# qiaozhijian/VCR-Net

Hardware: AMD Instinct MI355X
Metric: point-cloud pairs/sec (N=1024, batch 16 per GPU) (higher is better)
Workload: dtype f32; 1 GPU; BASELINE configs[1]: ModelNet40-like whole-to-whole registration, N=1024, batch=16 pairs per GPU, LPDNet(k=20)+Transformer+VcpTopK+SVD, iter=1, fp32; synthetic object clouds with the reference's transform recipe; LPD-pretrained emb_nn + seeded Transformer weights; num_points=1024, batch_per_gpu=16, global_batch=16, k=20, iters=1, parallelism=dp1 (pairs sharded per rank), entry_point=vcrnet_amd.module.vcrnetIter(net, src, tgt, iter) -> vcr_vcrnet_iter_f32

## Files before the change

### include/vcr_hip.h

```cpp
#ifndef VCR_HIP_H
#define VCR_HIP_H

#include <stddef.h>
#include <stdint.h>

#ifdef __cplusplus
extern "C" {
#endif

#define VCR_OK 0
#define VCR_EINVAL (-1)
#define VCR_EWORKSPACE (-2)
#define VCR_EUNSUPPORTED (-3)

typedef void* vcr_stream_t;

const char* vcr_strerror(int code);
#define VCR_ABI_VERSION 27
int vcr_abi_version(void);

typedef struct {
  const float* x_cf; int B, N;
  const float* w1; const float* b1;
  const float* w2; const float* b2;
  float* xyz4; float* feat64; float* sq64;
  const float* x_cf2; int B2;
  const float* pq_w; const float* pq_b; float* pq; int ldpq;
  float* feat64t;
} vcr_pointwise_args;
int vcr_pointwise_f32(const vcr_pointwise_args*, vcr_stream_t);

int vcr_rows4_f32(const float* x_cf, float* xyz4, int B, int N, vcr_stream_t);
int vcr_rows4_pq_f32(const float* x_cf, float* xyz4, int B, int N, const float* wpq, int ldw, const float* bpq, int C,
                     float* pq, int ldpq, vcr_stream_t);

typedef struct {
  uint32_t struct_bytes;
  const float* x; int ldx;
  const float* sq;
  int B, N, C, k;
  int32_t* idx;
  int32_t* tie_scratch; int tie_cap;
  int waves;
  int tie_zeroed;
  int tie_defer;
  void* tie_work; size_t tie_work_bytes;
  int tie_inline;
  const float* xt;
  const int32_t* perm; const float* xp; const float* sqp;
  const float* cen; const float* cen_sq; const float* cen_rad; const float* cen_sqmax;
  const int32_t* ord_ok;
} vcr_knn_args;

typedef struct {
  const float* xyz4;
  const float* feat_t; int ldf; const float* sq;
  int B, N;
  int32_t* perm; float* xyz4_p; float* cen4; float* cen4_rad; float* cen4_sqmax;
  float* feat_p; float* sq_p; float* cen64; float* cen64_sq; float* cen64_rad; float* cen64_sqmax;
  int32_t* ord_ok; float* ord_stat; float guard_ratio;
} vcr_knn_order_args;
int vcr_knn_order_f32(const vcr_knn_order_args*, vcr_stream_t);
int vcr_knn_f32(const vcr_knn_args*, vcr_stream_t);
size_t vcr_knn_tie_work_bytes(int N);
size_t vcr_knn_tie_slot_bytes(int B, int N);
int vcr_knn_ties_inline(const vcr_knn_args*);
int vcr_knn_ties_f32(const vcr_knn_args* a, const vcr_knn_args* b, vcr_stream_t);
int vcr_knn_pair_f32(const vcr_knn_args* a64, const vcr_knn_args* a3, vcr_stream_t);

typedef struct {
  const float* x; int ldx;
  const float* w;
  const float* bias;
  const float* residual; int ldr;
  float* y; int ldy;
  int M, N, K;
  int relu;
  const float* ln_stats_in; int ln_nseg; const float* ln_colsum; float ln_eps;
  float* stats_out;
  float* segmax_out; int ld_segmax; int seg_k;
  int variant;
} vcr_linear_args;
enum {
  VCR_LINEAR_REGSTAGE = 4, VCR_LINEAR_BK32 = 8, VCR_LINEAR_MFMA16 = 16, VCR_LINEAR_BK16 = 64, VCR_LINEAR_MFMA32 = 1024,
  VCR_LINEAR_ROWS96 = 2048, VCR_LINEAR_ROWS128 = 4096, VCR_LINEAR_ROWS64 = 8192, VCR_LINEAR_ROWS32 = 16384
};
int vcr_linear_f32(const vcr_linear_args*, vcr_stream_t);
int vcr_linear_config(const vcr_linear_args*);
int vcr_linear_pair_f32(const vcr_linear_args* a, const vcr_linear_args* b, vcr_stream_t);

int vcr_fold_layernorm_f32(const float* w, const float* bias, const float* ln_a, const float* ln_b, int N, int K,
                           float* w_out, float* colsum, float* bias_out, vcr_stream_t);

int vcr_split_bf16x3_f32(const float* x, void* planes, size_t n, vcr_stream_t);
int vcr_linear_bf16x3_f32(const vcr_linear_args*, const void* w_planes, vcr_stream_t);

typedef struct {
  const float* x; int ldx; const float* a; const float* b; float eps;
  const float* residual; int ldr;
  float* y; int ldy; int M, C;
  const float* xyz4; float* side4;
} vcr_layernorm_args;
int vcr_layernorm_f32(const vcr_layernorm_args*, vcr_stream_t);

typedef struct {
  const float* x; int ldx; int M, C; float scale; float* y; int ldy;
  const float* xyz4; float* side4;
} vcr_rowside_args;
int vcr_rowside_f32(const vcr_rowside_args*, vcr_stream_t);

typedef struct {
  const float* pq; int ldpq; const int32_t* idx; int k; int M; int n_per_cloud;
  const float* w2; const float* b2;
  float* x1; int ldx1; float* x2; int ldx2;
} vcr_edgeconv_args;
int vcr_edgeconv_f32(const vcr_edgeconv_args*, vcr_stream_t);
int vcr_edgeconv_bf16x3_f32(const vcr_edgeconv_args*, vcr_stream_t);

typedef struct {
  const float* pq; int ldpq; int C; const int32_t* idx; int k; int M; int n_per_cloud;
  float* y; int ldy;
  int variant;
  const int32_t* order;
} vcr_gathermax_args;
int vcr_gathermax_f32(const vcr_gathermax_args*, vcr_stream_t);

typedef struct {
  const float* pq; int ldpq; int C; const int32_t* idx; int k; int M; int n_per_cloud; float* h; int ldh;
  float* ymax; int ldymax; int zero_to;
} vcr_edgerows_args;
int vcr_edgerows_f32(const vcr_edgerows_args*, vcr_stream_t);
typedef struct {
  const float* pq; int ldpq; const int32_t* idx; int k; int M; int n_per_cloud;
  const float *w2, *b2, *w3, *b3, *w4, *b4;
  float* out; int ldo;
} vcr_edgechain_args;
int vcr_edgechain_f32(const vcr_edgechain_args*, vcr_stream_t);
typedef struct {
  const float* x; int ldx; int M, k, C; float* y; int ldy;
} vcr_segmax_args;
int vcr_segmax_f32(const vcr_segmax_args*, vcr_stream_t);

typedef struct {
  const float* q; int ldq; const float* k; int ldk; const float* v; int ldv;
  float* out; int ldo;
  int nbatch, heads, nq, nk; float scale; int kv_batch_shift;
  const uint8_t* key_keep; float* rowstat;
  float* score_out; int ld_score;
  int ngroups; long q_group_stride, k_group_stride, v_group_stride, out_group_stride;
  const int32_t* key_index; int nk_src;
  float* split_work; long split_work_floats;
  int variant;
  int plan_nbatch;
} vcr_sdpa_args;
#define VCR_SDPA_MAX_SPLIT 4
int vcr_sdpa_f32(const vcr_sdpa_args*, vcr_stream_t);
int vcr_sdpa_bf16x3_f32(const vcr_sdpa_args*, vcr_stream_t);

typedef struct {
  const float* score; int ld; int nbatch, heads, nq, nk;
  const float* rowstat; int q_batch_shift; float* mass;
} vcr_keymass_args;
int vcr_keymass_f32(const vcr_keymass_args*, vcr_stream_t);

typedef struct {
  const float* q; int ldq; const float* k; int ldk; const float* qside4; const float* kside4;
  float* corr4; int nbatch, nq, nk, E; int mode; float scale;
  float* split_work;
  long split_work_floats;
} vcr_softcorr_args;
int vcr_softcorr_f32(const vcr_softcorr_args*, vcr_stream_t);

typedef struct {
  const float* own; int ld_own; const float* str; int ld_str;
  const float* own_side4; const float* str_side4;
  int nbatch, n_own, n_str, E; int score; float scale; int str_batch_shift; int op;
  float* corr4; float* stat2; int32_t* argmax;
  const float* str_stat2; long str_stat_batch_stride; float* mass; int accumulate;
  float* score_out; int ld_score;
  int variant;
  float* split_work; long split_work_floats;
} vcr_pairscore_args;
#define VCR_PAIRSCORE_MAX_SPLIT 4
int vcr_pairscore_f32(const vcr_pairscore_args*, vcr_stream_t);

typedef struct {
  const float* score; int ld; int nbatch, n_rows, n_cols;
  const float* row_stat2; float* col_stat2; float* col_mass; float* row_mass;
} vcr_scoremass_args;
int vcr_scoremass_f32(const vcr_scoremass_args*, vcr_stream_t);

typedef struct {
  const float* values; int nbatch, n, K; int32_t* order; uint8_t* mask;
  int largest;
  int stride;
} vcr_rankselect_args;
int vcr_rankselect_f32(const vcr_rankselect_args*, vcr_stream_t);

typedef struct {
  const float* in; int ld_in; int n_in; const int32_t* idx; int nbatch, n_out, C; float* out; int ld_out;
  const int32_t* via; int n_via;
} vcr_gather_args;
int vcr_gather_rows_f32(const vcr_gather_args*, vcr_stream_t);

typedef struct {
  const float* src; int lds; const float* corr; int ldc; int B, K;
  float* R; float* t; float* R_ba; float* t_ba; float* H;
} vcr_rigid_svd_args;
int vcr_rigid_svd_f32(const vcr_rigid_svd_args*, vcr_stream_t);

typedef struct {
  const float* src4; const float* dst4; int B, N, M; int max_iterations; float tolerance;
  float* final4; float* R; float* t; float* R_ba; float* t_ba; int* iterations;
} vcr_icp_args;
size_t vcr_icp_workspace_bytes(int B, int N);
int vcr_icp_f32(const vcr_icp_args*, void* workspace, size_t workspace_bytes, vcr_stream_t);

typedef struct {
  const float* cloud; int P;
  const double* R_ab; const double* t_ab;
  const int32_t* pick; const int32_t* perm_src; const int32_t* perm_tgt;
  int B, N, keep;
  float* src_cf; float* tgt_cf;
} vcr_make_pairs_args;
int vcr_make_pairs_f32(const vcr_make_pairs_args*, vcr_stream_t);

typedef struct {
  uint32_t struct_bytes;
  const float* xyz_cf; long cloud_stride;
  int B, N, npoint;
  const int32_t* start;
  int32_t* idx;
  float* out_cf;
  int variant;
} vcr_fps_args;
int vcr_fps_f32(const vcr_fps_args*, vcr_stream_t);
int vcr_fps_form(const vcr_fps_args*, int* form, int* points_per_thread);

// ... 102 lines not shown
```

### vcr-net_amd/csrc/linear.hip

```cpp
#include "common.h"
#include "vcr_internal.h"
#include <type_traits>
#include <utility>

namespace {

constexpr int BM = 128, BN = 128;
constexpr int LINEAR_WG_PER_CU_BK32 = 2, LINEAR_WG_PER_CU_BK16 = 4;
constexpr int LINEAR_MS_DEFAULT = 0;


constexpr int LINEAR_BLOCKED_ACC = 0;

template <int BK> struct TileT { float a[BM][BK + 4]; float b[BN][BK + 4]; };

template <int BK>
__global__ __launch_bounds__(256, (BK == 32 ? 2 : 3)) void linear_kernel(vcr_linear_args p, int tiles_m, int tiles_n,
                                                                        int vec_epilogue) {
  using Tile = TileT<BK>;
  constexpr int CPR = BK / 4;
  constexpr int RPP = 256 / CPR;
  constexpr int NPASS = BM / RPP;
  extern __shared__ __attribute__((aligned(16))) unsigned char smem[];
  Tile* tile = reinterpret_cast<Tile*>(smem);
  const int t = threadIdx.x, lane = t & 63, wave = __builtin_amdgcn_readfirstlane(t >> 6);
  const int half = lane >> 5, l31 = lane & 31;
  const int wm = wave >> 1, wn = wave & 1;

  const int nblk = tiles_m * tiles_n;
  int bid = blockIdx.x;
  bid = xcd_chunk(bid, nblk);
  const int tm = bid / tiles_n, tn = bid % tiles_n;
  const int m0 = tm * BM, n0 = tn * BN;

  const int r0 = t / CPR, c4 = (t % CPR) * 4;
  const float* xa[NPASS];
  const float* wb[NPASS];
#pragma unroll
  for (int i = 0; i < NPASS; ++i) {
    xa[i] = p.x + (size_t)min(m0 + r0 + RPP * i, p.M - 1) * p.ldx + c4;
    wb[i] = p.w + (size_t)min(n0 + r0 + RPP * i, p.N - 1) * p.K + c4;
  }
  f32x4 ra[NPASS], rb[NPASS];
#pragma unroll
  for (int i = 0; i < NPASS; ++i) { ra[i] = ld4(xa[i]); rb[i] = ld4(wb[i]); }
#pragma unroll
  for (int i = 0; i < NPASS; ++i) { st4(&tile[0].a[r0 + RPP * i][c4], ra[i]); st4(&tile[0].b[r0 + RPP * i][c4], rb[i]); }
  __syncthreads();

  f32x16 acc[2][2];
#pragma unroll
  for (int i = 0; i < 2; ++i)
#pragma unroll
    for (int j = 0; j < 2; ++j) acc[i][j] = f32x16{0};

  f32x16 tot[2][2];
#pragma unroll
  for (int i = 0; i < 2; ++i)
#pragma unroll
    for (int j = 0; j < 2; ++j) tot[i][j] = f32x16{0};
  const int nk = p.K / BK;
  for (int kt = 0; kt < nk; ++kt) {
    const int cur = kt & 1;
    if (kt + 1 < nk) {
#pragma unroll
      for (int i = 0; i < NPASS; ++i) { ra[i] = ld4(xa[i] + (kt + 1) * BK); rb[i] = ld4(wb[i] + (kt + 1) * BK); }
    }
    const Tile& T = tile[cur];
#pragma unroll
    for (int g = 0; g < BK / 8; ++g) {
      f32x4 fa[2], fb[2];
#pragma unroll
      for (int i = 0; i < 2; ++i) fa[i] = ld4(&T.a[wm * 64 + i * 32 + l31][8 * g + 4 * half]);
#pragma unroll
      for (int j = 0; j < 2; ++j) fb[j] = ld4(&T.b[wn * 64 + j * 32 + l31][8 * g + 4 * half]);
#pragma unroll
      for (int s = 0; s < 4; ++s)
#pragma unroll
        for (int i = 0; i < 2; ++i)
#pragma unroll
          for (int j = 0; j < 2; ++j) acc[i][j] = mfma32(fa[i][s], fb[j][s], acc[i][j]);
    }
    if (LINEAR_BLOCKED_ACC && (((kt + 1) * BK) % 128 == 0 || kt + 1 == nk)) {
#pragma unroll
      for (int i = 0; i < 2; ++i)
#pragma unroll
        for (int j = 0; j < 2; ++j) { tot[i][j] += acc[i][j]; acc[i][j] = f32x16{0}; }
    }
    if (kt + 1 < nk) {
      Tile& Nx = tile[cur ^ 1];
#pragma unroll
      for (int i = 0; i < NPASS; ++i) { st4(&Nx.a[r0 + RPP * i][c4], ra[i]); st4(&Nx.b[r0 + RPP * i][c4], rb[i]); }
    }
    __syncthreads();
  }
  if (LINEAR_BLOCKED_ACC) {
#pragma unroll
    for (int i = 0; i < 2; ++i)
#pragma unroll
      for (int j = 0; j < 2; ++j) acc[i][j] = tot[i][j];
  }

  if (vec_epilogue) {
    constexpr int EP = 68;
    float* ot = reinterpret_cast<float*>(smem) + wave * 32 * EP;
    const int c4e = (lane & 15) * 4, col = n0 + wn * 64 + c4e;
    const f32x4 bias = (p.bias && col < p.N) ? ld4(p.bias + col) : f32x4{0.f, 0.f, 0.f, 0.f};
#pragma unroll
    for (int i = 0; i < 2; ++i) {
#pragma unroll
      for (int j = 0; j < 2; ++j)
#pragma unroll
        for (int r = 0; r < 16; ++r) ot[acc_row(r, half) * EP + j * 32 + l31] = acc[i][j][r];
      __builtin_amdgcn_s_waitcnt(0xc07f);
      __builtin_amdgcn_wave_barrier();
      if (col < p.N) {
#pragma unroll 4
        for (int ps = 0; ps < 8; ++ps) {
          const int rl = ps * 4 + (lane >> 4);
          const int row = m0 + wm * 64 + i * 32 + rl;
          if (row < p.M) {
            f32x4 v = ld4(&ot[rl * EP + c4e]) + bias;
            if (p.relu) v = f32x4{fmaxf(v[0], 0.f), fmaxf(v[1], 0.f), fmaxf(v[2], 0.f), fmaxf(v[3], 0.f)};
            if (p.residual) v = v + ld4(p.residual + (size_t)row * p.ldr + col);
            st4(p.y + (size_t)row * p.ldy + col, v);
          }
        }
      }
      __builtin_amdgcn_s_waitcnt(0xc07f);
      __builtin_amdgcn_wave_barrier();
    }
    return;
  }
#pragma unroll
  for (int j = 0; j < 2; ++j) {
    const int col = n0 + wn * 64 + j * 32 + l31;
    if (col >= p.N) continue;
    const float bias = p.bias ? p.bias[col] : 0.f;
#pragma unroll
    for (int i = 0; i < 2; ++i) {
#pragma unroll
      for (int r = 0; r < 16; ++r) {
        const int row = m0 + wm * 64 + i * 32 + acc_row(r, half);
        if (row < p.M) {
          float v = acc[i][j][r] + bias;
          if (p.relu) v = fmaxf(v, 0.f);
          if (p.residual) v += p.residual[(size_t)row * p.ldr + col];
          p.y[(size_t)row * p.ldy + col] = v;
        }
      }
    }
  }
}

template <int BK, int BMV = BM> struct TileGT { float a[BMV][BK]; float b[BN][BK]; };

__device__ __forceinline__ void glds16(const float* g, float* l) {
  __builtin_amdgcn_global_load_lds((const __attribute__((address_space(1))) void*)g,
                                   (__attribute__((address_space(3))) void*)l, 16, 0, 0);
}

template <int BK, int MS, int BMV = BM>
__device__ __forceinline__ void linear_glds_body(const vcr_linear_args& p, int tiles_m, int tiles_n, int blk) {
  const bool LN_IN = p.ln_stats_in != nullptr, STATS_OUT = p.stats_out != nullptr;
  static_assert(BMV == 128 || ((BMV == 96 || BMV == 64 || BMV == 32) && MS == 16), "the lower tiles are built from 16 x 16 MFMA tiles");
  using Tile = TileGT<BK, BMV>;
  constexpr int WR = BMV / 2;
  constexpr int EPR = BMV == 128 ? 32 : 16;
  constexpr int NPASS = WR / EPR, NPS = EPR / 4;
  constexpr int CPR = BK / 4;
  constexpr int RPK = 64 / CPR;
  constexpr int NF = 32 / RPK;
  constexpr int SWS = BK == 32 ? 1 : 2;
  constexpr int EP = 68;
  constexpr int STAGE_BYTES = 2 * sizeof(Tile) > 4 * 32 * EP * 4 ? 2 * sizeof(Tile) : 4 * 32 * EP * 4;
  extern __shared__ __attribute__((aligned(16))) unsigned char smem[];
  Tile* tile = reinterpret_cast<Tile*>(smem);
  float* rowst = reinterpret_cast<float*>(smem + STAGE_BYTES);
  const int t = threadIdx.x, lane = t & 63, wave = __builtin_amdgcn_readfirstlane(t >> 6);
  const int half = lane >> 5, l31 = lane & 31;
  const int wm = wave >> 1, wn = wave & 1;
  const int nblk = tiles_m * tiles_n;
  const int bid = xcd_chunk(blk, nblk);
  constexpr int GW = 12;
  const int grp = bid / (GW * tiles_m), wg = min(GW, tiles_n - grp * GW), loc = bid - grp * GW * tiles_m;
  const int tm = loc / wg, tn = grp * GW + loc % wg;
  const int m0 = tm * BMV, n0 = tn * BN;
  const int frow = lane / CPR, fpc = lane % CPR;
  constexpr int NFA = BMV == 128 ? NF : (BMV / RPK + 3) / 4;
  const float* xa[NFA];
  const float* wb[NF];
  int arow[NFA];
#pragma unroll
  for (int i = 0; i < NFA; ++i) {
    arow[i] = BMV == 128 ? wave * 32 + RPK * i : (wave + 4 * i) * RPK;
    const int row = min(arow[i], BMV - RPK) + frow;
    const int lc = fpc ^ ((row >> SWS) & (CPR - 1));
    xa[i] = p.x + (size_t)min(m0 + row, p.M - 1) * p.ldx + 4 * lc;
  }
#pragma unroll
  for (int i = 0; i < NF; ++i) {
    const int row = wave * 32 + RPK * i + frow;
    const int lc = fpc ^ ((row >> SWS) & (CPR - 1));
    wb[i] = p.w + (size_t)min(n0 + row, p.N - 1) * p.K + 4 * lc;
  }
  auto fill = [&](int buf, int k0) {
#pragma unroll
    for (int i = 0; i < NFA; ++i)
      if (BMV == 128 || arow[i] < BMV) glds16(xa[i] + k0, &tile[buf].a[min(arow[i], BMV - RPK)][0]);
#pragma unroll
    for (int i = 0; i < NF; ++i) glds16(wb[i] + k0, &tile[buf].b[wave * 32 + RPK * i][0]);
  };
  fill(0, 0);
  if (LN_IN && t < BMV) {
    float mean, var;
    ln_row_moments(p.ln_stats_in + (size_t)min(m0 + t, p.M - 1) * p.ln_nseg * 2, p.ln_nseg, p.K, mean, var);
    rowst[2 * t] = mean;
    rowst[2 * t + 1] = 1.f / (sqrtf(var) + p.ln_eps);
  }
  __syncthreads();

  constexpr int NT = MS == 32 ? 2 : 4;
  constexpr int NTM = WR / MS;
  const int qtr = lane >> 4, l15 = lane & 15;
  f32x16 acc[2][2];
  f32x4 acc4[MS == 16 ? NTM : 4][4];
#pragma unroll
  for (int i = 0; i < 2; ++i)
#pragma unroll
    for (int j = 0; j < 2; ++j) acc[i][j] = f32x16{0};
#pragma unroll
  for (int i = 0; i < (MS == 16 ? NTM : 4); ++i)
#pragma unroll
    for (int j = 0; j < 4; ++j) acc4[i][j] = f32x4{0.f, 0.f, 0.f, 0.f};
  int ra_[NT], rb_[NT], sa[NT], sb[NT];
#pragma unroll
  for (int i = 0; i < NT; ++i) {
    ra_[i] = wm * WR + i * MS + (MS == 32 ? l31 : l15); sa[i] = (ra_[i] >> SWS) & (CPR - 1);
    rb_[i] = wn * 64 + i * MS + (MS == 32 ? l31 : l15); sb[i] = (rb_[i] >> SWS) & (CPR - 1);
  }
  constexpr bool PREFETCH_RES = BK == 32;
  f32x4 resv[PREFETCH_RES ? NPASS : 1][PREFETCH_RES ? NPS : 1];
  if (PREFETCH_RES) {
    const int colr = n0 + wn * 64 + (lane & 15) * 4;
#pragma unroll
    for (int i = 0; i < NPASS; ++i)
#pragma unroll
      for (int ps = 0; ps < NPS; ++ps) {
        const int row = m0 + wm * WR + i * EPR + ps * 4 + (lane >> 4);
        resv[PREFETCH_RES ? i : 0][PREFETCH_RES ? ps : 0] =
            (p.residual && row < p.M && colr < p.N) ? ld4(p.residual + (size_t)row * p.ldr + colr) : f32x4{0.f, 0.f, 0.f, 0.f};
      }
  }
  constexpr bool BLOCKED = LINEAR_BLOCKED_ACC == 1 || (LINEAR_BLOCKED_ACC == 2 && BK == 32);
  f32x16 tot[BLOCKED ? 2 : 1][BLOCKED ? 2 : 1];
  f32x4 tot4[BLOCKED ? (MS == 16 ? NTM : 4) : 1][BLOCKED ? 4 : 1];
  if constexpr (BLOCKED) {
#pragma unroll
    for (int i = 0; i < 2; ++i)
#pragma unroll
      for (int j = 0; j < 2; ++j) tot[i][j] = f32x16{0};
#pragma unroll
    for (int i = 0; i < (MS == 16 ? NTM : 4); ++i)
#pragma unroll
      for (int j = 0; j < 4; ++j) tot4[i][j] = f32x4{0.f, 0.f, 0.f, 0.f};
  }
  auto bank = [&]() {
    if constexpr (BLOCKED) {
      if constexpr (MS == 32) {
#pragma unroll
        for (int i = 0; i < 2; ++i)
#pragma unroll
          for (int j = 0; j < 2; ++j) { tot[i][j] += acc[i][j]; acc[i][j] = f32x16{0}; }
      } else {
#pragma unroll
        for (int i = 0; i < NTM; ++i)
#pragma unroll
          for (int j = 0; j < 4; ++j) { tot4[i][j] += acc4[i][j]; acc4[i][j] = f32x4{0.f, 0.f, 0.f, 0.f}; }
      }
    }
  };
  const int nk = p.K / BK;
  for (int kt = 0; kt < nk; ++kt) {
    const int cur = kt & 1;
    if (kt + 1 < nk) fill(cur ^ 1, (kt + 1) * BK);
    const Tile& T = tile[cur];
    if constexpr (MS == 32) {
#pragma unroll
      for (int g = 0; g < BK / 8; ++g) {
        f32x4 fa[2], fb[2];
#pragma unroll
        for (int i = 0; i < 2; ++i) fa[i] = ld4(&T.a[ra_[i]][4 * ((2 * g + half) ^ sa[i])]);
#pragma unroll
        for (int j = 0; j < 2; ++j) fb[j] = ld4(&T.b[rb_[j]][4 * ((2 * g + half) ^ sb[j])]);
#pragma unroll
        for (int s = 0; s < 4; ++s)
#pragma unroll
          for (int i = 0; i < 2; ++i)
#pragma unroll
            for (int j = 0; j < 2; ++j) acc[i][j] = mfma32(fa[i][s], fb[j][s], acc[i][j]);
      }
    } else {
#pragma unroll
      for (int g = 0; g < BK / 16; ++g) {
        f32x4 fa[NTM], fb[4];
#pragma unroll
        for (int i = 0; i < NTM; ++i) fa[i] = ld4(&T.a[ra_[i]][4 * ((4 * g + qtr) ^ sa[i])]);
#pragma unroll
        for (int j = 0; j < 4; ++j) fb[j] = ld4(&T.b[rb_[j]][4 * ((4 * g + qtr) ^ sb[j])]);
#pragma unroll
        for (int s = 0; s < 4; ++s)
#pragma unroll
          for (int i = 0; i < NTM; ++i)
#pragma unroll
            for (int j = 0; j < 4; ++j) acc4[i][j] = mfma16(fa[i][s], fb[j][s], acc4[i][j]);
      }
    }
    if (BLOCKED && ((kt + 1) * BK) % 128 == 0 && kt + 1 < nk) bank();
    __syncthreads();
  }
  if constexpr (BLOCKED) {
    bank();
    if constexpr (MS == 32) {
#pragma unroll
      for (int i = 0; i < 2; ++i)
#pragma unroll
        for (int j = 0; j < 2; ++j) acc[i][j] = tot[i][j];
    } else {
#pragma unroll
      for (int i = 0; i < NTM; ++i)
#pragma unroll
        for (int j = 0; j < 4; ++j) acc4[i][j] = tot4[i][j];
    }
  }

  float* ot = reinterpret_cast<float*>(smem) + wave * 32 * EP;
  const int c4e = (lane & 15) * 4, col = n0 + wn * 64 + c4e;
  const f32x4 bias = (p.bias && col < p.N) ? ld4(p.bias + col) : f32x4{0.f, 0.f, 0.f, 0.f};
  const f32x4 csum = (LN_IN && col < p.N) ? ld4(p.ln_colsum + col) : f32x4{0.f, 0.f, 0.f, 0.f};
  int run_pt = -1;
  f32x4 run_mx = {0.f, 0.f, 0.f, 0.f};
  auto seg_flush = [&]() {
    if (run_pt >= 0 && (lane >> 4) == 0 && col < p.N) {
      int* o = reinterpret_cast<int*>(p.segmax_out + (size_t)run_pt * p.ld_segmax + col);
#pragma unroll
      for (int e = 0; e < 4; ++e) atomicMax(o + e, __float_as_int(run_mx[e]));
    }
    run_pt = -1;
  };
#pragma unroll
  for (int i = 0; i < NPASS; ++i) {
    if constexpr (MS == 32) {
#pragma unroll
      for (int j = 0; j < 2; ++j)
#pragma unroll
        for (int r = 0; r < 16; ++r) ot[acc_row(r, half) * EP + j * 32 + l31] = acc[i][j][r];
    } else {
#pragma unroll
      for (int ih = 0; ih < EPR / 16; ++ih)
#pragma unroll
        for (int jt = 0; jt < 4; ++jt)
#pragma unroll
          for (int r = 0; r < 4; ++r) ot[(16 * ih + 4 * qtr + r) * EP + jt * 16 + l15] = acc4[EPR / 16 * i + ih][jt][r];
    }
    __builtin_amdgcn_s_waitcnt(0xc07f);
    __builtin_amdgcn_wave_barrier();
    if (p.segmax_out) {
#pragma unroll
      for (int ps = 0; ps < NPS; ++ps) {
        const int rl = ps * 4 + (lane >> 4);
        const int row0 = m0 + wm * WR + i * EPR + ps * 4, row = row0 + (lane >> 4);
        f32x4 v = ld4(&ot[rl * EP + c4e]) + bias;
        v = f32x4{fmaxf(v[0], 0.f), fmaxf(v[1], 0.f), fmaxf(v[2], 0.f), fmaxf(v[3], 0.f)};
        if (row >= p.M || col >= p.N) v = f32x4{0.f, 0.f, 0.f, 0.f};
        else if (p.y) st4(p.y + (size_t)row * p.ldy + col, v);
        if (row0 >= p.M) continue;
        const int pa = row0 / p.seg_k, pb = min(row0 + 3, p.M - 1) / p.seg_k;
        if (pa == pb) {
#pragma unroll
          for (int e = 0; e < 4; ++e) {
            v[e] = fmaxf(v[e], __shfl_xor(v[e], 16, 64));
            v[e] = fmaxf(v[e], __shfl_xor(v[e], 32, 64));
          }
          if (pa != run_pt) { seg_flush(); run_pt = pa; run_mx = v; }
          else {
#pragma unroll
            for (int e = 0; e < 4; ++e) run_mx[e] = fmaxf(run_mx[e], v[e]);
          }
        } else {
          seg_flush();
          if (row < p.M && col < p.N) {
            int* o = reinterpret_cast<int*>(p.segmax_out + (size_t)(row / p.seg_k) * p.ld_segmax + col);
#pragma unroll
            for (int e = 0; e < 4; ++e) atomicMax(o + e, __float_as_int(v[e]));
          }
        }
      }
      if (i == NPASS - 1) seg_flush();
    } else if (col < p.N) {
#pragma unroll
      for (int ps = 0; ps < NPS; ++ps) {
        const int rl = ps * 4 + (lane >> 4);
        const int row = m0 + wm * WR + i * EPR + rl;
        if (row < p.M) {
          f32x4 v = ld4(&ot[rl * EP + c4e]);
          if (LN_IN) {
            const float mean = rowst[2 * (wm * WR + i * EPR + rl)], inv = rowst[2 * (wm * WR + i * EPR + rl) + 1];
#pragma unroll
            for (int e = 0; e < 4; ++e) v[e] = fmaf(inv, fmaf(-mean, csum[e], v[e]), bias[e]);
          } else {
            v = v + bias;
          }
          if (p.relu) v = f32x4{fmaxf(v[0], 0.f), fmaxf(v[1], 0.f), fmaxf(v[2], 0.f), fmaxf(v[3], 0.f)};
          if (p.residual) v = v + (PREFETCH_RES ? resv[PREFETCH_RES ? i : 0][PREFETCH_RES ? ps : 0]
                                                : ld4(p.residual + (size_t)row * p.ldr + col));
          st4(p.y + (size_t)row * p.ldy + col, v);
          if (STATS_OUT) {
            float s1 = (v[0] + v[1]) + (v[2] + v[3]);
            s1 = row16_sum(s1);
            const float ms = s1 * (1.f / 64.f);
            const float d0 = v[0] - ms, d1 = v[1] - ms, d2 = v[2] - ms, d3 = v[3] - ms;
            float s2 = (d0 * d0 + d1 * d1) + (d2 * d2 + d3 * d3);
            s2 = row16_sum(s2);
            if ((lane & 15) == 0) {
              float* so = p.stats_out + ((size_t)row * (p.N / 64) + (n0 + wn * 64) / 64) * 2;
              so[0] = s1; so[1] = s2;
            }
          }
        }
      }
    }
    __builtin_amdgcn_s_waitcnt(0xc07f);
    __builtin_amdgcn_wave_barrier();
  }
}

template <int BK, int MS, int BMV>
__global__ __launch_bounds__(256, (BK == 32 ? LINEAR_WG_PER_CU_BK32 : LINEAR_BLOCKED_ACC == 1 ? 3 : LINEAR_WG_PER_CU_BK16)) void linear_glds_kernel(vcr_linear_args p, int tiles_m, int tiles_n) {
  linear_glds_body<BK, MS, BMV>(p, tiles_m, tiles_n, (int)blockIdx.x);
}
template <int BK, int MS, int BMV>
__global__ __launch_bounds__(256, (BK == 32 ? LINEAR_WG_PER_CU_BK32 : LINEAR_BLOCKED_ACC == 1 ? 3 : LINEAR_WG_PER_CU_BK16)) void linear_glds_pair_kernel(vcr_linear_args p0, vcr_linear_args p1, int tm0,
                                                                                 int tn0, int tm1, int tn1) {
  const int n0 = tm0 * tn0;
  if ((int)blockIdx.x < n0) linear_glds_body<BK, MS, BMV>(p0, tm0, tn0, (int)blockIdx.x);
  else linear_glds_body<BK, MS, BMV>(p1, tm1, tn1, (int)blockIdx.x - n0);
}

}

namespace {
struct LinearPlan { bool glds; int bk, ms, bm, tiles_m, tiles_n, vec, lds; };
struct LinearForced { int bk, ms, rows; bool any, rows_free; };
struct LinearHalf { const vcr_linear_args* a; int vec; bool glds; LinearForced v; };

constexpr int LINEAR_SMALL_M = 16384;
constexpr double LINEAR_ROWS96_MARGIN = 1.02;
constexpr int LINEAR_ROWS[4] = {128, 96, 64, 32};

int small_grid_rows(const long* tiles_by_h, int cus) {
  if (tiles_by_h[0] >= (long)LINEAR_WG_PER_CU_BK32 * cus) return 0;
  int best = 128;
  double bc = 1e30;
  for (int i = 0; i < 4; ++i) {
    const long per_cu = (tiles_by_h[i] + cus - 1) / cus;
    const double c = ((double)(per_cu / 2) * 1.75 + (double)(per_cu & 1)) * (LINEAR_ROWS[i] + 24);
    if (c < bc - 1e-9) { bc = c; best = LINEAR_ROWS[i]; }
  }
  return best;
}

double launch_cost(long tiles, int slots, int rows) {
  const long full = tiles / slots;
  const double f = (double)(tiles - full * slots) / slots;
  double c;
  if (full == 0) c = f <= 0.0 ? 0.0 : f <= 0.5 ? 0.6 : 1.0;
  else c = (double)full + (f <= 0.0 ? 0.0 : f <= 0.3 ? 0.5 : f >= 0.7 ? 1.0 : 0.5 + (f - 0.3) * 1.25);
  return c * rows;
}

int linear_check(const vcr_linear_args* a, LinearHalf* f) {
  if (!a || !a->x || !a->w || (!a->y && !a->segmax_out)) return VCR_EINVAL;
  if (a->segmax_out && (a->seg_k <= 0 || !a->relu || a->residual || a->ln_stats_in || a->stats_out || (a->ld_segmax & 3) ||
                        a->ld_segmax < a->N || ((uintptr_t)a->segmax_out & 15) || (a->variant & VCR_LINEAR_REGSTAGE)))
    return VCR_EINVAL;
  if (a->M <= 0 || a->N <= 0 || a->K <= 0 || (a->K % 32) != 0) return VCR_EINVAL;
  const int variant = a->variant;
  constexpr int ROWS64_32 = VCR_LINEAR_ROWS64 | VCR_LINEAR_ROWS32;
  if (variant & ~(VCR_LINEAR_REGSTAGE | VCR_LINEAR_BK32 | VCR_LINEAR_MFMA16 | VCR_LINEAR_BK16 | VCR_LINEAR_MFMA32 | VCR_LINEAR_ROWS96 |
                  VCR_LINEAR_ROWS128 | ROWS64_32))
    return VCR_EINVAL;
  if ((variant & VCR_LINEAR_ROWS96) && (variant & (VCR_LINEAR_ROWS128 | VCR_LINEAR_MFMA32 | VCR_LINEAR_REGSTAGE)))
    return VCR_EINVAL;
  if ((variant & ROWS64_32) && ((variant & (VCR_LINEAR_ROWS128 | VCR_LINEAR_ROWS96 | VCR_LINEAR_MFMA32 | VCR_LINEAR_BK16 | VCR_LINEAR_REGSTAGE)) ||
                                (variant & ROWS64_32) == ROWS64_32))
    return VCR_EINVAL;
  if ((a->ldx & 3) || a->ldx < a->K || (a->y && a->ldy < a->N) || (a->residual && a->ldr < a->N)) return VCR_EINVAL;
  if (((uintptr_t)a->x | (uintptr_t)a->w) & 15) return VCR_EINVAL;
  f->a = a;
  f->vec = (a->N % 4 == 0) && (!a->y || ((a->ldy % 4 == 0) && (((uintptr_t)a->y & 15) == 0))) &&
           (!a->bias || ((uintptr_t)a->bias & 15) == 0) &&
           (!a->residual || ((a->ldr % 4 == 0) && ((uintptr_t)a->residual & 15) == 0));
  if (a->ln_stats_in || a->stats_out) {
    if (a->ln_stats_in && (!a->ln_colsum || !a->bias || a->ln_nseg <= 0 || a->K < 2 || (a->K % a->ln_nseg))) return VCR_EINVAL;
    if (a->stats_out && (a->N % 64)) return VCR_EINVAL;
    if (!f->vec || (variant & VCR_LINEAR_REGSTAGE)) return VCR_EUNSUPPORTED;
    if (a->ln_stats_in && ((uintptr_t)a->ln_colsum & 15)) return VCR_EINVAL;
  }
  if (a->segmax_out && !f->vec) return VCR_EUNSUPPORTED;
  f->glds = !(variant & VCR_LINEAR_REGSTAGE) && f->vec;
  if ((variant & (VCR_LINEAR_ROWS96 | ROWS64_32)) && !f->glds) return VCR_EUNSUPPORTED;
  return VCR_OK;
}

LinearForced linear_forced(int variant) {
  return {(variant & VCR_LINEAR_BK32) ? 32 : (variant & VCR_LINEAR_BK16) ? 16 : 0,
          (variant & VCR_LINEAR_MFMA16) ? 16 : (variant & VCR_LINEAR_MFMA32) ? 32 : 0,
          (variant & VCR_LINEAR_ROWS96) ? 96 : (variant & VCR_LINEAR_ROWS128) ? 128 : (variant & VCR_LINEAR_ROWS64) ? 64 :
          (variant & VCR_LINEAR_ROWS32) ? 32 : 0,
          variant != 0, !(variant & (VCR_LINEAR_ROWS96 | VCR_LINEAR_ROWS128 | VCR_LINEAR_ROWS64 | VCR_LINEAR_ROWS32 | VCR_LINEAR_MFMA32))};
}

bool linear_plan(const LinearHalf* h, int n, LinearPlan* pl) {
  const int cus = vcr_cu_count();
  auto regular_rows = [&](bool bk32, const long* t) {
    const int slots = cus * (bk32 ? LINEAR_WG_PER_CU_BK32 : LINEAR_WG_PER_CU_BK16);
    return bk32 && LINEAR_ROWS96_MARGIN * launch_cost(t[1], slots, 96) < launch_cost(t[0], slots, 128) ? 96 : 128;
  };
  long total[4] = {0, 0, 0, 0};
  int bk[2], ms[2], rows[2];
  bool small_free[2], rows_free[2];
  for (int i = 0; i < n; ++i) {
    const vcr_linear_args& a = *h[i].a;
    const LinearForced& v = h[i].v;
    const int tiles_n = (a.N + BN - 1) / BN;
    long t[4];
    for (int j = 0; j < 4; ++j) { t[j] = (long)((a.M + LINEAR_ROWS[j] - 1) / LINEAR_ROWS[j]) * tiles_n; total[j] += t[j]; }
    const bool one_round16 = n == 1 && !v.any && a.M >= LINEAR_SMALL_M && a.K >= 512 && t[0] <= (long)LINEAR_WG_PER_CU_BK16 * cus;
    bk[i] = v.bk ? v.bk : (a.residual || one_round16) ? 32 : 16;
    small_free[i] = h[i].glds && !v.any && a.M < LINEAR_SMALL_M;
    ms[i] = v.ms ? v.ms : small_free[i] ? 16 : LINEAR_MS_DEFAULT ? LINEAR_MS_DEFAULT : bk[i] == 32 ? 16 : 32;
    rows_free[i] = h[i].glds && v.rows_free;
    rows[i] = v.rows ? v.rows : rows_free[i] ? regular_rows(bk[i] == 32, t) : BM;
    const int sr = small_free[i] ? small_grid_rows(t, cus) : 0;
    if (sr && sr < 96) rows[i] = sr;
  }
  if (n == 2) {
    int joint = small_free[0] && small_free[1] ? small_grid_rows(total, cus) : 0;
    if (joint >= 96 || (joint == 0 && rows_free[0] && rows_free[1])) {
      const bool r = h[0].a->residual != nullptr, rb = h[1].a->residual != nullptr;
      joint = r == rb ? regular_rows(r, total) : 0;
    }
    if (joint) rows[0] = rows[1] = joint;
  }
  static_assert(2 * sizeof(TileGT<16>) == 2 * (BM + BN) * 16 * 4 && 2 * sizeof(TileGT<32, 96>) == 2 * (96 + BN) * 32 * 4, "stage size below");
  for (int i = 0; i < n; ++i) {
    const vcr_linear_args& a = *h[i].a;
    const bool glds = h[i].glds;
    const int bm = rows[i];
    if (!glds || bm < 96) bk[i] = 32;
    ms[i] = !glds ? 32 : bm < 128 ? 16 : ms[i];
    const int stage = 2 * (bm + BN) * bk[i] * 4, epi = 4 * 32 * 68 * 4;
    pl[i] = LinearPlan{glds, bk[i], ms[i], bm, (a.M + bm - 1) / bm, (a.N + BN - 1) / BN, h[i].vec,
                       glds ? (stage > epi ? stage : epi) + (a.ln_stats_in ? bm * 2 * 4 : 0) : (int)(2 * sizeof(TileT<32>))};
  }
  if (n == 1) return true;
  if (pl[0].glds && pl[1].glds && pl[0].bk == pl[1].bk && pl[0].ms == pl[1].ms && pl[0].bm == pl[1].bm && !h[0].a->segmax_out &&
      !h[1].a->segmax_out) {
    pl[0].lds = pl[1].lds = pl[0].lds > pl[1].lds ? pl[0].lds : pl[1].lds;
    return true;
  }
  linear_plan(h, 1, pl);
  linear_plan(h + 1, 1, pl + 1);
  return false;
}

int linear_prepare(const vcr_linear_args* a, const vcr_linear_args* b, int n, LinearPlan* pl, bool* one_launch) {
  const vcr_linear_args* args[2] = {a, b};
  LinearHalf h[2];
  for (int i = 0; i < n; ++i) {
    const int rc = linear_check(args[i], &h[i]);
    if (rc != VCR_OK) return rc;
    h[i].v = linear_forced(args[i]->variant);
  }
  *one_launch = linear_plan(h, n, pl);
  return VCR_OK;
}

template <class F>
void linear_dispatch(const LinearPlan& pl, F&& f) {
  using I16 = std::integral_constant<int, 16>; using I32 = std::integral_constant<int, 32>; using I64 = std::integral_constant<int, 64>;
  using I96 = std::integral_constant<int, 96>; using I128 = std::integral_constant<int, 128>;
  const bool bk16 = pl.bk == 16, ms16 = pl.ms == 16;
  if (pl.bm == 64) f(I32{}, I16{}, I64{});
  else if (pl.bm == 32) f(I32{}, I16{}, I32{});
  else if (pl.bm == 96) { if (bk16) f(I16{}, I16{}, I96{}); else f(I32{}, I16{}, I96{}); }
  else if (bk16) { if (ms16) f(I16{}, I16{}, I128{}); else f(I16{}, I32{}, I128{}); }
  else { if (ms16) f(I32{}, I16{}, I128{}); else f(I32{}, I32{}, I128{}); }
}

int linear_launch(const LinearPlan& p, const vcr_linear_args& a, hipStream_t s) {
  const dim3 grid(p.tiles_m * p.tiles_n), block(256);
  int rc = 0;
  if (p.glds) linear_dispatch(p, [&](auto bk, auto ms, auto bm) {
    rc = vcr_launch<linear_glds_kernel<decltype(bk)::value, decltype(ms)::value, decltype(bm)::value>>(grid, block, p.lds, s, a, p.tiles_m, p.tiles_n);
  });
  else rc = vcr_launch<linear_kernel<32>>(grid, block, p.lds, s, a, p.tiles_m, p.tiles_n, p.vec);
  return rc;
}
int linear_launch(const LinearPlan& p, const vcr_linear_args& a, const LinearPlan& q, const vcr_linear_args& b, hipStream_t s) {
  const dim3 grid(p.tiles_m * p.tiles_n + q.tiles_m * q.tiles_n), block(256);
  int rc = 0;
  linear_dispatch(p, [&](auto bk, auto ms, auto bm) {
    rc = vcr_launch<linear_glds_pair_kernel<decltype(bk)::value, decltype(ms)::value, decltype(bm)::value>>(
        grid, block, p.lds, s, a, b, p.tiles_m, p.tiles_n, q.tiles_m, q.tiles_n);
  });
  return rc;
}
}

extern "C" int vcr_linear_forms_(const vcr_linear_args* a, const vcr_linear_args* b, int* one_launch, int* form_a, int* form_b) {
  LinearPlan pl[2];
  bool one;
  const int n = b ? 2 : 1, rc = linear_prepare(a, b, n, pl, &one);
  if (rc != VCR_OK) return rc;
  if (one_launch) *one_launch = one;
  int* const forms[2] = {form_a, form_b};
  for (int i = 0; i < n; ++i)
    if (forms[i]) {
      const int f[8] = {pl[i].glds, pl[i].bm, pl[i].bk, pl[i].ms, pl[i].tiles_m, pl[i].tiles_n, pl[i].lds, pl[i].vec};
      memcpy(forms[i], f, sizeof(f));
    }
  return VCR_OK;
}

extern "C" int vcr_linear_config(const vcr_linear_args* a) {
  int f[8];
  const int rc = vcr_linear_forms_(a, nullptr, nullptr, f, nullptr);
  return rc != VCR_OK ? rc : f[1] | (f[2] << 8) | (f[3] == 16 ? 1 << 16 : 0) | (f[0] ? 1 << 17 : 0);
}

extern "C" int vcr_linear_f32(const vcr_linear_args* a, vcr_stream_t stream) {
  vcr_stream_scope bound(stream);
  LinearPlan pl;
  bool one;
  const int rc = linear_prepare(a, nullptr, 1, &pl, &one);
  return rc != VCR_OK ? rc : linear_launch(pl, *a, (hipStream_t)stream);
}

extern "C" int vcr_linear_pair_f32(const vcr_linear_args* a, const vcr_linear_args* b, vcr_stream_t stream) {
  vcr_stream_scope bound(stream);
  LinearPlan pl[2];
  bool one;
  int rc = linear_prepare(a, b, 2, pl, &one);
  if (rc != VCR_OK) return rc;
  hipStream_t s = (hipStream_t)stream;
  if (one) return linear_launch(pl[0], *a, pl[1], *b, s);
  rc = linear_launch(pl[0], *a, s);
  return rc ? rc : linear_launch(pl[1], *b, s);
}
```

Measured before the change: 3217 pairs/s.

## Add register-resident epilogue for glds linear kernel, skipping LDS staging

Adds a REGEPI path to the global-load-LDS linear kernel. MFMA operands are swapped so each lane holds contiguous column quads of the output, which lets bias, layernorm correction, relu, residual and the store happen straight from accumulators instead of round-tripping through LDS. Per-row segment statistics are reduced with permlane swap instructions. It is enabled by default for BK32/MFMA16 tiles other than 96 rows. It adds new kernel instantiations and inline asm, and it changes the reduction order of the stats output.

```diff
diff --git a/include/vcr_hip.h b/include/vcr_hip.h
--- a/include/vcr_hip.h
+++ b/include/vcr_hip.h
@@ -83,7 +83,8 @@
 } vcr_linear_args;
 enum {
   VCR_LINEAR_REGSTAGE = 4, VCR_LINEAR_BK32 = 8, VCR_LINEAR_MFMA16 = 16, VCR_LINEAR_BK16 = 64, VCR_LINEAR_MFMA32 = 1024,
-  VCR_LINEAR_ROWS96 = 2048, VCR_LINEAR_ROWS128 = 4096, VCR_LINEAR_ROWS64 = 8192, VCR_LINEAR_ROWS32 = 16384
+  VCR_LINEAR_ROWS96 = 2048, VCR_LINEAR_ROWS128 = 4096, VCR_LINEAR_ROWS64 = 8192, VCR_LINEAR_ROWS32 = 16384,
+  VCR_LINEAR_EPI_LDS = 32768, VCR_LINEAR_EPI_REG = 65536
 };
 int vcr_linear_f32(const vcr_linear_args*, vcr_stream_t);
 int vcr_linear_config(const vcr_linear_args*);
diff --git a/vcr-net_amd/csrc/linear.hip b/vcr-net_amd/csrc/linear.hip
--- a/vcr-net_amd/csrc/linear.hip
+++ b/vcr-net_amd/csrc/linear.hip
@@ -160,7 +160,23 @@
                                    (__attribute__((address_space(3))) void*)l, 16, 0, 0);
 }
 
-template <int BK, int MS, int BMV = BM>
+__device__ __forceinline__ float stat_leaf(const f32x4& v) { return (v[0] + v[1]) + (v[2] + v[3]); }
+__device__ __forceinline__ float stat_leaf_dev(const f32x4& v, float ms) {
+  const float d0 = v[0] - ms, d1 = v[1] - ms, d2 = v[2] - ms, d3 = v[3] - ms;
+  return (d0 * d0 + d1 * d1) + (d2 * d2 + d3 * d3);
+}
+__device__ __forceinline__ float xor32_sum(float v) {
+  float w = v;
+  asm volatile("s_nop 1\n\tv_permlane32_swap_b32 %0, %1" : "+v"(v), "+v"(w));
+  return v + w;
+}
+__device__ __forceinline__ float xor16_sum(float v) {
+  float w = v;
+  asm volatile("s_nop 1\n\tv_permlane16_swap_b32 %0, %1" : "+v"(v), "+v"(w));
+  return v + w;
+}
+
+template <int BK, int MS, int BMV = BM, bool REGEPI = false>
 __device__ __forceinline__ void linear_glds_body(const vcr_linear_args& p, int tiles_m, int tiles_n, int blk) {
   const bool LN_IN = p.ln_stats_in != nullptr, STATS_OUT = p.stats_out != nullptr;
   static_assert(BMV == 128 || ((BMV == 96 || BMV == 64 || BMV == 32) && MS == 16), "the lower tiles are built from 16 x 16 MFMA tiles");
@@ -240,15 +256,33 @@
     rb_[i] = wn * 64 + i * MS + (MS == 32 ? l31 : l15); sb[i] = (rb_[i] >> SWS) & (CPR - 1);
   }
   constexpr bool PREFETCH_RES = BK == 32;
-  f32x4 resv[PREFETCH_RES ? NPASS : 1][PREFETCH_RES ? NPS : 1];
-  if (PREFETCH_RES) {
+  constexpr int RQ = MS == 32 ? 32 : 16, CQW = MS == 32 ? 8 : 16, NRI = WR / RQ, NCQ = 64 / CQW;
+  const int rl0 = wm * WR + (MS == 32 ? l31 : l15), cl0 = wn * 64 + 4 * (MS == 32 ? half : qtr);
+  f32x4 resq[PREFETCH_RES && REGEPI ? NRI : 1][PREFETCH_RES && REGEPI ? NCQ : 1];
+  if constexpr (PREFETCH_RES && REGEPI) {
+#pragma unroll
+    for (int i = 0; i < NRI; ++i)
+#pragma unroll
+      for (int cq = 0; cq < NCQ; ++cq) {
+        const int row = m0 + rl0 + RQ * i, colr = n0 + cl0 + CQW * cq;
+        resq[i][cq] = (p.residual && row < p.M && colr < p.N) ? ld4(p.residual + (size_t)row * p.ldr + colr) : f32x4{0.f, 0.f, 0.f, 0.f};
+      }
+  }
+  f32x4 bcq = {0.f, 0.f, 0.f, 0.f};
+  if constexpr (REGEPI) {
+    const float* src = lane < 16 ? p.bias : LN_IN ? p.ln_colsum : nullptr;
+    const int colb = n0 + wn * 64 + 4 * (lane & 15);
+    if (lane < 32 && src && colb < p.N) bcq = ld4(src + colb);
+  }
+  f32x4 resv[PREFETCH_RES && !REGEPI ? NPASS : 1][PREFETCH_RES && !REGEPI ? NPS : 1];
+  if constexpr (PREFETCH_RES && !REGEPI) {
     const int colr = n0 + wn * 64 + (lane & 15) * 4;
 #pragma unroll
     for (int i = 0; i < NPASS; ++i)
 #pragma unroll
       for (int ps = 0; ps < NPS; ++ps) {
         const int row = m0 + wm * WR + i * EPR + ps * 4 + (lane >> 4);
-        resv[PREFETCH_RES ? i : 0][PREFETCH_RES ? ps : 0] =
+        resv[i][ps] =
             (p.residual && row < p.M && colr < p.N) ? ld4(p.residual + (size_t)row * p.ldr + colr) : f32x4{0.f, 0.f, 0.f, 0.f};
       }
   }
@@ -298,7 +332,7 @@
 #pragma unroll
           for (int i = 0; i < 2; ++i)
 #pragma unroll
-            for (int j = 0; j < 2; ++j) acc[i][j] = mfma32(fa[i][s], fb[j][s], acc[i][j]);
+            for (int j = 0; j < 2; ++j) acc[i][j] = REGEPI ? mfma32(fb[j][s], fa[i][s], acc[i][j]) : mfma32(fa[i][s], fb[j][s], acc[i][j]);
       }
     } else {
 #pragma unroll
@@ -313,7 +347,7 @@
 #pragma unroll
           for (int i = 0; i < NTM; ++i)
 #pragma unroll
-            for (int j = 0; j < 4; ++j) acc4[i][j] = mfma16(fa[i][s], fb[j][s], acc4[i][j]);
+            for (int j = 0; j < 4; ++j) acc4[i][j] = REGEPI ? mfma16(fb[j][s], fa[i][s], acc4[i][j]) : mfma16(fa[i][s], fb[j][s], acc4[i][j]);
       }
     }
     if (BLOCKED && ((kt + 1) * BK) % 128 == 0 && kt + 1 < nk) bank();
@@ -334,6 +368,90 @@
     }
   }
 
+  if constexpr (REGEPI) {
+    auto quad = [&](int i, int cq) -> f32x4 {
+      if constexpr (MS == 32) {
+        const f32x16& a = acc[i][cq >> 2];
+        const int g = cq & 3;
+        return f32x4{a[4 * g], a[4 * g + 1], a[4 * g + 2], a[4 * g + 3]};
+      } else {
+        return acc4[i][cq];
+      }
+    };
+    auto set_quad = [&](int i, int cq, const f32x4& v) {
+      if constexpr (MS == 32) {
+        const int g = cq & 3;
+#pragma unroll
+        for (int e = 0; e < 4; ++e) acc[i][cq >> 2][4 * g + e] = v[e];
+      } else {
+        acc4[i][cq] = v;
+      }
+    };
+    float* bl = reinterpret_cast<float*>(smem) + wave * 32 * EP;
+    if (lane < 32) st4(bl + 4 * lane, bcq);
+    __builtin_amdgcn_s_waitcnt(0xc07f);
+    __builtin_amdgcn_wave_barrier();
+    {
+      const bool LN = LN_IN, RELU = p.relu != 0, RES = p.residual != nullptr;
+#pragma unroll
+      for (int it = 0; it < 2 * NRI; ++it) {
+        const int i = it % NRI, line = it / NRI;
+        const int row = m0 + rl0 + RQ * i;
+        const float mean = LN ? rowst[2 * (rl0 + RQ * i)] : 0.f, inv = LN ? rowst[2 * (rl0 + RQ * i) + 1] : 0.f;
+#pragma unroll
+        for (int cq = line * (NCQ / 2); cq < (line + 1) * (NCQ / 2); ++cq) {
+          const int cl = cl0 - wn * 64 + CQW * cq, col = n0 + wn * 64 + cl;
+          const f32x4 bias = ld4(bl + cl);
+          f32x4 v = quad(i, cq);
+          if (LN) {
+            const f32x4 csum = ld4(bl + 64 + cl);
+#pragma unroll
+            for (int e = 0; e < 4; ++e) v[e] = fmaf(inv, fmaf(-mean, csum[e], v[e]), bias[e]);
+          } else {
+            v = v + bias;
+          }
+          if (RELU) v = f32x4{fmaxf(v[0], 0.f), fmaxf(v[1], 0.f), fmaxf(v[2], 0.f), fmaxf(v[3], 0.f)};
+          if (row < p.M && col < p.N) {
+            if (RES) v = v + (PREFETCH_RES ? resq[PREFETCH_RES ? i : 0][PREFETCH_RES ? cq : 0]
+                                                     : ld4(p.residual + (size_t)row * p.ldr + col));
+            st4(p.y + (size_t)row * p.ldy + col, v);
+          }
+          set_quad(i, cq, v);
+        }
+        __builtin_amdgcn_sched_barrier(0);
+      }
+    }
+    if (STATS_OUT && n0 + wn * 64 < p.N) {
+#pragma unroll
+      for (int i = 0; i < NRI; ++i) {
+        const int row = m0 + rl0 + RQ * i;
+        auto tree = [&](auto leaf, float& sa, float& sb) {
+          float Q[4];
+          if constexpr (MS == 32) {
+            float P[8];
+#pragma unroll
+            for (int cq = 0; cq < 8; ++cq) P[cq] = xor32_sum(leaf(cq, cq >> 1));
+#pragma unroll
+            for (int q = 0; q < 4; ++q) Q[q] = P[2 * q] + P[2 * q + 1];
+          } else {
+#pragma unroll
+            for (int q = 0; q < 4; ++q) Q[q] = xor32_sum(xor16_sum(leaf(q, q)));
+          }
+          sa = (Q[0] + Q[3]) + (Q[1] + Q[2]);
+          sb = (Q[0] + Q[1]) + (Q[2] + Q[3]);
+        };
+        float s1a, s1b, s2a, s2b;
+        tree([&](int cq, int) { return stat_leaf(quad(i, cq)); }, s1a, s1b);
+        const float msa = s1a * (1.f / 64.f), msb = s1b * (1.f / 64.f);
+        tree([&](int cq, int q) { return stat_leaf_dev(quad(i, cq), (q & 1) ? msb : msa); }, s2a, s2b);
+        if (row < p.M && (MS == 32 ? half : qtr) == 0) {
+          float* so = p.stats_out + ((size_t)row * (p.N / 64) + (n0 + wn * 64) / 64) * 2;
+          so[0] = s1a; so[1] = s2a;
+        }
+      }
+    }
+    return;
+  }
   float* ot = reinterpret_cast<float*>(smem) + wave * 32 * EP;
   const int c4e = (lane & 15) * 4, col = n0 + wn * 64 + c4e;
   const f32x4 bias = (p.bias && col < p.N) ? ld4(p.bias + col) : f32x4{0.f, 0.f, 0.f, 0.f};
@@ -412,16 +530,13 @@
             v = v + bias;
           }
           if (p.relu) v = f32x4{fmaxf(v[0], 0.f), fmaxf(v[1], 0.f), fmaxf(v[2], 0.f), fmaxf(v[3], 0.f)};
-          if (p.residual) v = v + (PREFETCH_RES ? resv[PREFETCH_RES ? i : 0][PREFETCH_RES ? ps : 0]
+          if (p.residual) v = v + (PREFETCH_RES ? resv[PREFETCH_RES && !REGEPI ? i : 0][PREFETCH_RES && !REGEPI ? ps : 0]
                                                 : ld4(p.residual + (size_t)row * p.ldr + col));
           st4(p.y + (size_t)row * p.ldy + col, v);
           if (STATS_OUT) {
-            float s1 = (v[0] + v[1]) + (v[2] + v[3]);
-            s1 = row16_sum(s1);
+            const float s1 = row16_sum(stat_leaf(v));
             const float ms = s1 * (1.f / 64.f);
-            const float d0 = v[0] - ms, d1 = v[1] - ms, d2 = v[2] - ms, d3 = v[3] - ms;
-            float s2 = (d0 * d0 + d1 * d1) + (d2 * d2 + d3 * d3);
-            s2 = row16_sum(s2);
+            const float s2 = row16_sum(stat_leaf_dev(v, ms));
             if ((lane & 15) == 0) {
               float* so = p.stats_out + ((size_t)row * (p.N / 64) + (n0 + wn * 64) / 64) * 2;
               so[0] = s1; so[1] = s2;
@@ -446,12 +561,23 @@
   if ((int)blockIdx.x < n0) linear_glds_body<BK, MS, BMV>(p0, tm0, tn0, (int)blockIdx.x);
   else linear_glds_body<BK, MS, BMV>(p1, tm1, tn1, (int)blockIdx.x - n0);
 }
+template <int BK, int MS, int BMV>
+__global__ __launch_bounds__(256, (BK == 32 ? LINEAR_WG_PER_CU_BK32 : LINEAR_BLOCKED_ACC == 1 ? 3 : LINEAR_WG_PER_CU_BK16)) void linear_glds_reg_kernel(vcr_linear_args p, int tiles_m, int tiles_n) {
+  linear_glds_body<BK, MS, BMV, true>(p, tiles_m, tiles_n, (int)blockIdx.x);
+}
+template <int BK, int MS, int BMV>
+__global__ __launch_bounds__(256, (BK == 32 ? LINEAR_WG_PER_CU_BK32 : LINEAR_BLOCKED_ACC == 1 ? 3 : LINEAR_WG_PER_CU_BK16)) void linear_glds_reg_pair_kernel(vcr_linear_args p0, vcr_linear_args p1, int tm0,
+                                                                                     int tn0, int tm1, int tn1) {
+  const int n0 = tm0 * tn0;
+  if ((int)blockIdx.x < n0) linear_glds_body<BK, MS, BMV, true>(p0, tm0, tn0, (int)blockIdx.x);
+  else linear_glds_body<BK, MS, BMV, true>(p1, tm1, tn1, (int)blockIdx.x - n0);
+}
 
 }
 
 namespace {
-struct LinearPlan { bool glds; int bk, ms, bm, tiles_m, tiles_n, vec, lds; };
-struct LinearForced { int bk, ms, rows; bool any, rows_free; };
+struct LinearPlan { bool glds; int bk, ms, bm, tiles_m, tiles_n, vec, lds; bool reg; };
+struct LinearForced { int bk, ms, rows; bool any, rows_free; int epi; };
 struct LinearHalf { const vcr_linear_args* a; int vec; bool glds; LinearForced v; };
 
 constexpr int LINEAR_SMALL_M = 16384;
@@ -479,6 +605,11 @@
   return c * rows;
 }
 
+bool linear_epilogue_reg(int bk, int ms, int rows, bool residual, bool stats) {
+  (void)residual; (void)stats;
+  return bk == 32 && ms == 16 && rows != 96;
+}
+
 int linear_check(const vcr_linear_args* a, LinearHalf* f) {
   if (!a || !a->x || !a->w || (!a->y && !a->segmax_out)) return VCR_EINVAL;
   if (a->segmax_out && (a->seg_k <= 0 || !a->relu || a->residual || a->ln_stats_in || a->stats_out || (a->ld_segmax & 3) ||
@@ -486,9 +617,11 @@
     return VCR_EINVAL;
   if (a->M <= 0 || a->N <= 0 || a->K <= 0 || (a->K % 32) != 0) return VCR_EINVAL;
   const int variant = a->variant;
-  constexpr int ROWS64_32 = VCR_LINEAR_ROWS64 | VCR_LINEAR_ROWS32;
+  constexpr int ROWS64_32 = VCR_LINEAR_ROWS64 | VCR_LINEAR_ROWS32, EPI = VCR_LINEAR_EPI_LDS | VCR_LINEAR_EPI_REG;
   if (variant & ~(VCR_LINEAR_REGSTAGE | VCR_LINEAR_BK32 | VCR_LINEAR_MFMA16 | VCR_LINEAR_BK16 | VCR_LINEAR_MFMA32 | VCR_LINEAR_ROWS96 |
-                  VCR_LINEAR_ROWS128 | ROWS64_32))
+                  VCR_LINEAR_ROWS128 | ROWS64_32 | EPI))
+    return VCR_EINVAL;
+  if ((variant & EPI) == EPI || ((variant & VCR_LINEAR_EPI_REG) && ((variant & VCR_LINEAR_REGSTAGE) || a->segmax_out)))
     return VCR_EINVAL;
   if ((variant & VCR_LINEAR_ROWS96) && (variant & (VCR_LINEAR_ROWS128 | VCR_LINEAR_MFMA32 | VCR_LINEAR_REGSTAGE)))
     return VCR_EINVAL;
@@ -509,16 +642,18 @@
   }
   if (a->segmax_out && !f->vec) return VCR_EUNSUPPORTED;
   f->glds = !(variant & VCR_LINEAR_REGSTAGE) && f->vec;
-  if ((variant & (VCR_LINEAR_ROWS96 | ROWS64_32)) && !f->glds) return VCR_EUNSUPPORTED;
+  if ((variant & (VCR_LINEAR_ROWS96 | ROWS64_32 | VCR_LINEAR_EPI_REG)) && !f->glds) return VCR_EUNSUPPORTED;
   return VCR_OK;
 }
 
 LinearForced linear_forced(int variant) {
+  const int epi = (variant & VCR_LINEAR_EPI_LDS) ? 1 : (variant & VCR_LINEAR_EPI_REG) ? 2 : 0;
+  variant &= ~(VCR_LINEAR_EPI_LDS | VCR_LINEAR_EPI_REG);
   return {(variant & VCR_LINEAR_BK32) ? 32 : (variant & VCR_LINEAR_BK16) ? 16 : 0,
           (variant & VCR_LINEAR_MFMA16) ? 16 : (variant & VCR_LINEAR_MFMA32) ? 32 : 0,
           (variant & VCR_LINEAR_ROWS96) ? 96 : (variant & VCR_LINEAR_ROWS128) ? 128 : (variant & VCR_LINEAR_ROWS64) ? 64 :
           (variant & VCR_LINEAR_ROWS32) ? 32 : 0,
-          variant != 0, !(variant & (VCR_LINEAR_ROWS96 | VCR_LINEAR_ROWS128 | VCR_LINEAR_ROWS64 | VCR_LINEAR_ROWS32 | VCR_LINEAR_MFMA32))};
+          variant != 0, !(variant & (VCR_LINEAR_ROWS96 | VCR_LINEAR_ROWS128 | VCR_LINEAR_ROWS64 | VCR_LINEAR_ROWS32 | VCR_LINEAR_MFMA32)), epi};
 }
 
 bool linear_plan(const LinearHalf* h, int n, LinearPlan* pl) {
@@ -561,12 +696,15 @@
     if (!glds || bm < 96) bk[i] = 32;
     ms[i] = !glds ? 32 : bm < 128 ? 16 : ms[i];
     const int stage = 2 * (bm + BN) * bk[i] * 4, epi = 4 * 32 * 68 * 4;
+    const bool reg = glds && !a.segmax_out &&
+                     (h[i].v.epi ? h[i].v.epi == 2 : linear_epilogue_reg(bk[i], ms[i], bm, a.residual != nullptr, a.stats_out != nullptr));
     pl[i] = LinearPlan{glds, bk[i], ms[i], bm, (a.M + bm - 1) / bm, (a.N + BN - 1) / BN, h[i].vec,
-                       glds ? (stage > epi ? stage : epi) + (a.ln_stats_in ? bm * 2 * 4 : 0) : (int)(2 * sizeof(TileT<32>))};
+                       glds ? (stage > epi ? stage : epi) + (a.ln_stats_in ? bm * 2 * 4 : 0) : (int)(2 * sizeof(TileT<32>)), reg};
   }
   if (n == 1) return true;
-  if (pl[0].glds && pl[1].glds && pl[0].bk == pl[1].bk && pl[0].ms == pl[1].ms && pl[0].bm == pl[1].bm && !h[0].a->segmax_out &&
-      !h[1].a->segmax_out) {
+  if (pl[0].reg != pl[1].reg && !h[0].v.epi && !h[1].v.epi) pl[0].reg = pl[1].reg = false;
+  if (pl[0].glds && pl[1].glds && pl[0].bk == pl[1].bk && pl[0].ms == pl[1].ms && pl[0].bm == pl[1].bm && pl[0].reg == pl[1].reg &&
+      !h[0].a->segmax_out && !h[1].a->segmax_out) {
     pl[0].lds = pl[1].lds = pl[0].lds > pl[1].lds ? pl[0].lds : pl[1].lds;
     return true;
   }
@@ -603,7 +741,9 @@
   const dim3 grid(p.tiles_m * p.tiles_n), block(256);
   int rc = 0;
   if (p.glds) linear_dispatch(p, [&](auto bk, auto ms, auto bm) {
-    rc = vcr_launch<linear_glds_kernel<decltype(bk)::value, decltype(ms)::value, decltype(bm)::value>>(grid, block, p.lds, s, a, p.tiles_m, p.tiles_n);
+    constexpr int BK_ = decltype(bk)::value, MS_ = decltype(ms)::value, BM_ = decltype(bm)::value;
+    rc = p.reg ? vcr_launch<linear_glds_reg_kernel<BK_, MS_, BM_>>(grid, block, p.lds, s, a, p.tiles_m, p.tiles_n)
+               : vcr_launch<linear_glds_kernel<BK_, MS_, BM_>>(grid, block, p.lds, s, a, p.tiles_m, p.tiles_n);
   });
   else rc = vcr_launch<linear_kernel<32>>(grid, block, p.lds, s, a, p.tiles_m, p.tiles_n, p.vec);
   return rc;
@@ -612,8 +752,9 @@
   const dim3 grid(p.tiles_m * p.tiles_n + q.tiles_m * q.tiles_n), block(256);
   int rc = 0;
   linear_dispatch(p, [&](auto bk, auto ms, auto bm) {
-    rc = vcr_launch<linear_glds_pair_kernel<decltype(bk)::value, decltype(ms)::value, decltype(bm)::value>>(
-        grid, block, p.lds, s, a, b, p.tiles_m, p.tiles_n, q.tiles_m, q.tiles_n);
+    constexpr int BK_ = decltype(bk)::value, MS_ = decltype(ms)::value, BM_ = decltype(bm)::value;
+    rc = p.reg ? vcr_launch<linear_glds_reg_pair_kernel<BK_, MS_, BM_>>(grid, block, p.lds, s, a, b, p.tiles_m, p.tiles_n, q.tiles_m, q.tiles_n)
+               : vcr_launch<linear_glds_pair_kernel<BK_, MS_, BM_>>(grid, block, p.lds, s, a, b, p.tiles_m, p.tiles_n, q.tiles_m, q.tiles_n);
   });
   return rc;
 }
@@ -635,9 +776,10 @@
 }
 
 extern "C" int vcr_linear_config(const vcr_linear_args* a) {
-  int f[8];
-  const int rc = vcr_linear_forms_(a, nullptr, nullptr, f, nullptr);
-  return rc != VCR_OK ? rc : f[1] | (f[2] << 8) | (f[3] == 16 ? 1 << 16 : 0) | (f[0] ? 1 << 17 : 0);
+  LinearPlan pl;
+  bool one;
+  const int rc = linear_prepare(a, nullptr, 1, &pl, &one);
+  return rc != VCR_OK ? rc : pl.bm | (pl.bk << 8) | (pl.ms == 16 ? 1 << 16 : 0) | (pl.glds ? 1 << 17 : 0) | (pl.reg ? 1 << 18 : 0);
 }
 
 extern "C" int vcr_linear_f32(const vcr_linear_args* a, vcr_stream_t stream) {
```

Result: no change. 3215 pairs/s (-0.0%).
